# GatorSense/HyperPRI

Hardware: AMD Instinct MI355X
Metric: HSI cubes/sec (608x968x238) fwd+bwd (higher is better)
Workload: dtype f32; 1 GPU; CubeNET-64 n_channels=238 HSI 608x968 fp32, per-GPU batch 2, train mode, BCEWithLogits, fwd+bwd; global_batch=2, parallelism=dp1

## Files before the change

### hyperpri_amd/csrc/common.h

```cpp
#pragma once
#include <hip/hip_runtime.h>
#include <stdint.h>

#define HPRI_OK 0
#define HPRI_ERR_ARG (-1)
#define HPRI_ERR_UNSUPPORTED (-2)
#define HPRI_ERR_WORKSPACE (-3)
#define HPRI_ERR_LAUNCH (-4)

#ifdef HPRI_H16_F16
typedef _Float16 h16_t;
#define HPRI_MFMA_16X16X32 __builtin_amdgcn_mfma_f32_16x16x32_f16
#define HPRI_MFMA_32X32X16 __builtin_amdgcn_mfma_f32_32x32x16_f16
#define HPRI_DS_READ_TR16_B64 __builtin_amdgcn_ds_read_tr16_b64_v4f16
#define HPRI_H16_IS_F16 1
#else
typedef __bf16 h16_t;
#define HPRI_MFMA_16X16X32 __builtin_amdgcn_mfma_f32_16x16x32_bf16
#define HPRI_MFMA_32X32X16 __builtin_amdgcn_mfma_f32_32x32x16_bf16
#define HPRI_DS_READ_TR16_B64 __builtin_amdgcn_ds_read_tr16_b64_v4bf16
#define HPRI_H16_IS_F16 0
#endif

#ifdef HPRI_H16_F16
typedef __fp16 hpri_tr4_t __attribute__((__vector_size__(4 * sizeof(__fp16))));
#else
typedef __bf16 hpri_tr4_t __attribute__((ext_vector_type(4)));
#endif
typedef hpri_tr4_t __attribute__((address_space(3))) * hpri_lds_tr4_ptr;

typedef float f32x16 __attribute__((ext_vector_type(16)));
typedef float f32x4 __attribute__((ext_vector_type(4)));

#define HPRI_CHECK_LAUNCH()                                   \
  do {                                                        \
    hipError_t e__ = hipGetLastError();                       \
    if (e__ != hipSuccess) return hpri_set_error(HPRI_ERR_LAUNCH, hipGetErrorString(e__)); \
  } while (0)

#define HPRI_REQUIRE(cond, msg)                               \
  do {                                                        \
    if (!(cond)) return hpri_set_error(HPRI_ERR_ARG, msg);    \
  } while (0)

int hpri_set_error(int code, const char* msg);
int hpri_option(int idx);
int hpri_cu_count();
float hpri_loss_scale();

static inline int hpri_cdiv(int a, int b) { return (a + b - 1) / b; }
static inline int64_t hpri_cdiv64(int64_t a, int64_t b) { return (a + b - 1) / b; }

enum { HPRI_A_DIRECT = 0, HPRI_A_S2D = 1 };
enum { HPRI_E_DIRECT = 0, HPRI_E_D2S = 1 };

typedef h16_t bf16x4_t __attribute__((ext_vector_type(4)));
struct PlaneOut { h16_t* p; long long plane; int cs, coff, cw, npl; };

#ifdef __HIPCC__
__device__ __forceinline__ void plane_store4(const PlaneOut& pl, size_t pix, int c, float o0, float o1, float o2, float o3) {
  float v[4] = {o0, o1, o2, o3};
  for (int k = 0; k < pl.npl; ++k) {
    bf16x4_t h;
#pragma unroll
    for (int j = 0; j < 4; ++j) { const h16_t t = (h16_t)v[j]; h[j] = t; v[j] -= (float)t; }
    *reinterpret_cast<bf16x4_t*>(pl.p + (size_t)k * pl.plane + pix * pl.cs + pl.coff + c) = h;
  }
}
#endif

#define HPRI_DMA_OOB 0xFFFFFFF0u
#if defined(__HIP_DEVICE_COMPILE__)
typedef __amdgpu_buffer_rsrc_t hpri_rsrc_t;
#define HPRI_MAKE_RSRC(ptr_, bytes_) __builtin_amdgcn_make_buffer_rsrc((void*)(ptr_), 0, (int)(bytes_), 0x00020000)
#define HPRI_LDS_DMA16(rs_, lds_, voff_, soff_) \
  __builtin_amdgcn_raw_ptr_buffer_load_lds(rs_, (__attribute__((address_space(3))) void*)(lds_), 16, voff_, soff_, 0, 0)
#define HPRI_BUFFER_LOAD_F32(rs_, voff_, soff_) __builtin_bit_cast(float, __builtin_amdgcn_raw_buffer_load_b32(rs_, voff_, soff_, 0))
typedef unsigned hpri_u32x4 __attribute__((ext_vector_type(4)));
#define HPRI_BUFFER_LOAD_F32X4(rs_, voff_, soff_) __builtin_bit_cast(f32x4, __builtin_amdgcn_raw_buffer_load_b128(rs_, voff_, soff_, 0))
#define HPRI_BUFFER_STORE_F32X4(v_, rs_, voff_, soff_) \
  __builtin_amdgcn_raw_buffer_store_b128(__builtin_bit_cast(hpri_u32x4, v_), rs_, voff_, soff_, 0)
#else
typedef int hpri_rsrc_t;
#define HPRI_MAKE_RSRC(ptr_, bytes_) 0
#define HPRI_LDS_DMA16(rs_, lds_, voff_, soff_) ((void)(rs_))
#define HPRI_BUFFER_LOAD_F32(rs_, voff_, soff_) 0.f
#define HPRI_BUFFER_LOAD_F32X4(rs_, voff_, soff_) (f32x4{0.f, 0.f, 0.f, 0.f})
#define HPRI_BUFFER_STORE_F32X4(v_, rs_, voff_, soff_) ((void)(rs_))
#endif

#define HPRI_Q_SLICES 8
#define HPRI_Q_STRIDE 1024
#define HPRI_Q_COUNTERS (8 * HPRI_Q_SLICES)
#define HPRI_Q_HALF (HPRI_Q_COUNTERS * HPRI_Q_STRIDE)
#define HPRI_Q_WORDS (2 * HPRI_Q_HALF)
struct HpriQueueHalves { unsigned *use, *clear; };
HpriQueueHalves hpri_item_queue_take(hipStream_t stream);
#ifdef __HIPCC__
__device__ __forceinline__ unsigned hpri_q_draw(unsigned* q, int band, unsigned n) {
  return __hip_atomic_fetch_add(q + band * HPRI_Q_STRIDE, n, __ATOMIC_RELAXED, __HIP_MEMORY_SCOPE_AGENT);
}
__device__ __forceinline__ void hpri_q_clear(unsigned* other, int tid) {
  if (other != nullptr && tid < HPRI_Q_COUNTERS) __hip_atomic_store(other + tid * HPRI_Q_STRIDE, 0u, __ATOMIC_RELAXED, __HIP_MEMORY_SCOPE_AGENT);
}
#endif

static inline int hpri_plane_out(PlaneOut* po, void* planes, long long plane_stride, int pl_cs, int pl_coff, int pl_cw, int npl, int C) {
  po->p = reinterpret_cast<h16_t*>(planes); po->plane = plane_stride; po->cs = pl_cs; po->coff = pl_coff; po->cw = pl_cw; po->npl = npl;
  if (planes == nullptr) { po->cw = 0; po->npl = 0; return HPRI_OK; }
  HPRI_REQUIRE(npl >= 1 && npl <= 3 && pl_cw >= C && pl_cw % 4 == 0 && pl_coff % 4 == 0 && pl_cs % 4 == 0 && pl_coff + pl_cw <= pl_cs &&
                   plane_stride % 4 == 0 && ((uintptr_t)planes & 7) == 0, "bad plane geometry");
  return HPRI_OK;
}
```

### hyperpri_amd/csrc/conv_wino.hip

```cpp
#include "common.h"

typedef float f32x2 __attribute__((ext_vector_type(2)));

extern "C" size_t hpri_wino_packed_floats(int K, int Ncols_pad) { return (size_t)hpri_cdiv(K, 8) * 16 * 8 * Ncols_pad; }

struct WinoWgradArgs {
  const float* x; int x_cs, x_coff, x_cvalid;
  const float* dy; int dy_cs, dy_coff, dy_cvalid;
  float* ws;
  int N, H, W, Cr, Nr, cblk;
  int strips_x, strips_y, total, per_split;
  int ntile, items, per_xcd;
  int kw;
};

#define WG_XROW 36
#define WG_X_BYTES (4 * WG_XROW * 256)
#define WG_Y_BYTES (2 * 32 * 256)
#define WG_STAGE_BYTES (WG_X_BYTES + WG_Y_BYTES)

__global__ __launch_bounds__(512, 2) void conv_wino_wgrad_kernel(WinoWgradArgs a) {
  __shared__ __attribute__((aligned(1024))) unsigned char smem[2 * WG_STAGE_BYTES];
  const int tid = threadIdx.x, lane = tid & 63, wave = __builtin_amdgcn_readfirstlane(tid >> 6);
  const int li = lane & 31, lh = lane >> 5;
  const int fa = wave >> 1, fb = wave & 1;
  const int item = (int)(blockIdx.x & 7) * a.per_xcd + (int)(blockIdx.x >> 3);
  if (item >= a.items) return;
  const int split = item / a.ntile, tile = item - split * a.ntile;
  const int cb = tile % a.cblk, nbk = tile / a.cblk;
  const int c_blk = cb * 64, n_blk = nbk * 64;
  const int u0 = split * a.per_split, u1 = min(a.total, u0 + a.per_split);

  const float s1 = (fa == 2) ? -1.f : 1.f;

  f32x16 acc[2][2][2];
#pragma unroll
  for (int e = 0; e < 2; ++e)
#pragma unroll
    for (int ct = 0; ct < 2; ++ct)
#pragma unroll
      for (int nt = 0; nt < 2; ++nt)
#pragma unroll
        for (int r = 0; r < 16; ++r) acc[e][ct][nt][r] = 0.f;

  constexpr int NPX = 4 * (WG_XROW / 4), NPY = 2 * 8, NPW = (NPX + NPY + 7) / 8;
  constexpr unsigned OOB = 0xFFFFFFF0u;
  const int l4 = lane >> 4;
  const unsigned xlane = (c_blk + (lane & 15) * 4 < a.x_cvalid) ? (unsigned)(l4 * a.x_cs * 4 + (lane & 15) * 16) : OOB;
  const unsigned ylane = (n_blk + (lane & 15) * 4 < a.dy_cvalid) ? (unsigned)(l4 * a.dy_cs * 4 + (lane & 15) * 16) : OOB;
  int ld_sx = u0 % a.strips_x, ld_sy = (u0 / a.strips_x) % a.strips_y, ld_img = u0 / (a.strips_x * a.strips_y);
#define LOAD_UNIT(buf_)                                                                                                \
  {                                                                                                                    \
    const int sx_ = ld_sx, sy_ = ld_sy, img_ = ld_img;                                                                 \
    if (++ld_sx == a.strips_x) { ld_sx = 0; if (++ld_sy == a.strips_y) { ld_sy = 0; ++ld_img; } }                      \
    const int y0_ = sy_ * 2, x0_ = sx_ * 32;                                                                           \
    kend_next = min(8, (a.kw - x0_ + 3) >> 2);                                \
    unsigned char* lb_ = smem + (buf_) * WG_STAGE_BYTES;                                                               \
    const float* xu_ = a.x + ((long long)(img_ * a.H + y0_ - 1) * a.W + x0_ - 1) * a.x_cs + a.x_coff + c_blk;          \
    const float* yu_ = a.dy + ((long long)(img_ * a.H + y0_) * a.W + x0_) * a.dy_cs + a.dy_coff + n_blk;               \
    const hpri_rsrc_t rx_ = HPRI_MAKE_RSRC(xu_, 0x7FFFFF00);       \
    const hpri_rsrc_t ry_ = HPRI_MAKE_RSRC(yu_, 0x7FFFFF00);       \
    _Pragma("unroll") for (int p = 0; p < NPW; ++p) {                                                                  \
      const int piece_ = p * 8 + wave;                                                                                 \
      if (piece_ < NPX) {                                                                                              \
        const int row_ = piece_ / (WG_XROW / 4), pxb_ = (piece_ % (WG_XROW / 4)) * 4;                 \
        const bool rowok_ = (unsigned)(y0_ + row_ - 1) < (unsigned)a.H;                                                \
        const bool ok_ = rowok_ && (pxb_ + l4) < 34 && (unsigned)(x0_ + pxb_ + l4 - 1) < (unsigned)a.W;                \
        HPRI_LDS_DMA16(rx_, lb_ + piece_ * 1024, ok_ ? xlane : OOB, (row_ * a.W + pxb_) * a.x_cs * 4);           \
      } else if (piece_ < NPX + NPY) {                                                                                 \
        const int pp_ = piece_ - NPX;                                                                                  \
        const int row_ = pp_ >> 3, pxb_ = (pp_ & 7) * 4;                                                               \
        const bool ok_ = (y0_ + row_) < a.H && (x0_ + pxb_ + l4) < a.W;                                                \
        HPRI_LDS_DMA16(ry_, lb_ + piece_ * 1024, ok_ ? ylane : OOB, (row_ * a.W + pxb_) * a.dy_cs * 4);          \
      }                                                                                                                \
    }                                                                                                                  \
  }

#define K_STEP(FA_, FB_)                                               \
    {                                                                                                                  \
      constexpr int R1_ = (FA_ == 0) ? 0 : 1, R2_ = (FA_ == 3) ? 3 : 2;              \
      constexpr int YR_ = (FA_ == 3) ? 1 : 0, YROWS_ = (FA_ == 1 || FA_ == 2) ? 2 : 1;                                 \
      asm("" : "+v"(kp));                               \
      f32x2 d[2][3], y[2][2];                                          \
      _Pragma("unroll") for (int c = 0; c < 3; ++c) {                                                                  \
        d[0][c] = WG_LDS2(kp + (R1_ * WG_XROW + FB_ + c) * 256);                                                       \
        d[1][c] = WG_LDS2(kp + (R2_ * WG_XROW + FB_ + c) * 256);                                                       \
      }                                                                                                                \
      _Pragma("unroll") for (int r = 0; r < YROWS_; ++r)                                                               \
        _Pragma("unroll") for (int px = 0; px < 2; ++px) y[r][px] = WG_LDS2(kp + WG_X_BYTES + ((YR_ + r) * 32 + px) * 256); \
      float va[2][2], vb[2][2];                                               \
      float P[3][2];                                                                                                   \
      _Pragma("unroll") for (int c = 0; c < 3; ++c)                                                                    \
        _Pragma("unroll") for (int ct = 0; ct < 2; ++ct) {                                                             \
          float d1_ = d[0][c][ct], d2_ = d[1][c][ct];                                                                  \
          WG_PIN(d1_) WG_PIN(d2_)                                                                                      \
          P[c][ct] = (FA_ == 1) ? (d1_ + d2_) : (d1_ - d2_);                                        \
          WG_PIN(P[c][ct])                                                                                             \
        }                                                                                                              \
      _Pragma("unroll") for (int ct = 0; ct < 2; ++ct) {                                                               \
        va[0][ct] = FB_ ? (P[1][ct] - P[0][ct]) : (P[0][ct] - P[2][ct]);                                               \
        va[1][ct] = FB_ ? (P[0][ct] - P[2][ct]) : (P[1][ct] + P[2][ct]);                                               \
                                                                                                                       \
      }                                                                                                                \
      float t[2][2];                                                               \
      _Pragma("unroll") for (int px = 0; px < 2; ++px)                                                                 \
        _Pragma("unroll") for (int nt = 0; nt < 2; ++nt) {                                                             \
          float y0_ = y[0][px][nt];                                                                                    \
          WG_PIN(y0_)                                                                                                  \
          if (YROWS_ == 2) {                                                                                           \
            float y1_ = y[1][px][nt];                                                                                  \
            WG_PIN(y1_)                                                                                                \
            y0_ = (FA_ == 1) ? (y0_ + y1_) : (y0_ - y1_);                                                              \
            WG_PIN(y0_)                                                                                                \
          }                                                                                                            \
          t[px][nt] = y0_;                                                                                             \
        }                                                                                                              \
      _Pragma("unroll") for (int nt = 0; nt < 2; ++nt) {                                                               \
        vb[0][nt] = FB_ ? (t[0][nt] - t[1][nt]) : t[0][nt];                                                            \
        vb[1][nt] = FB_ ? t[1][nt] : (t[0][nt] + t[1][nt]);                                                            \
                                                                                                                       \
      }                                                                                                                \
      __builtin_amdgcn_sched_barrier(0);                            \
      _Pragma("unroll") for (int e = 0; e < 2; ++e)                                                                    \
          _Pragma("unroll") for (int ct = 0; ct < 2; ++ct)                                                             \
              _Pragma("unroll") for (int nt = 0; nt < 2; ++nt)                                                         \
                  acc[e][ct][nt] = __builtin_amdgcn_mfma_f32_32x32x2f32(va[e][ct], vb[e][nt], acc[e][ct][nt], 0, 0, 0); \
      kp += 1024;                                                                           \
    }
#define UNIT_LOOP(FA_, FB_)                                                                                            \
  for (int u = u0; u < u1; ++u) {                                                                                      \
    asm volatile("s_waitcnt vmcnt(0)" ::: "memory");                                                                   \
    __builtin_amdgcn_s_barrier();                     \
    const int kend = kend_next;                                                                                        \
    if (u + 1 < u1) LOAD_UNIT((u + 1 - u0) & 1)                                                                         \
    unsigned kp = ((u - u0) & 1) * WG_STAGE_BYTES + klane;                                                             \
    for (int kk = 0; kk < kend; ++kk) K_STEP(FA_, FB_)                                                                 \
  }
  const unsigned klane = (unsigned)(lh * 512 + li * 8);
  typedef __attribute__((address_space(3))) const unsigned char* wg_lds_bytes;
  typedef __attribute__((address_space(3))) const volatile f32x2* wg_lds_f32x2;
  const wg_lds_bytes lds = (wg_lds_bytes)smem;
#define WG_LDS2(off_) (*(wg_lds_f32x2)(lds + (off_)))
#define WG_PIN(v_) asm("" : "+v"(v_));
  int kend_next = 8;
  if (u0 < u1) LOAD_UNIT(0)
  switch (wave) {
    case 0: UNIT_LOOP(0, 0) break;
    case 1: UNIT_LOOP(0, 1) break;
    case 2: UNIT_LOOP(1, 0) break;
    case 3: UNIT_LOOP(1, 1) break;
    case 4: UNIT_LOOP(2, 0) break;
    case 5: UNIT_LOOP(2, 1) break;
    case 6: UNIT_LOOP(3, 0) break;
    default: UNIT_LOOP(3, 1) break;
  }
#undef UNIT_LOOP
#undef K_STEP
#undef LOAD_UNIT
#undef WG_LDS2
#undef WG_PIN
  float* slab = a.ws + (size_t)split * 16 * a.Cr * a.Nr;
  const float sdy = (fa == 3) ? -s1 : s1;
  const float sgn[2] = {sdy, (fb == 1) ? -sdy : sdy};
#pragma unroll
  for (int e = 0; e < 2; ++e) {
    const int xi = fa * 4 + 2 * fb + e;
#pragma unroll
    for (int ct = 0; ct < 2; ++ct)
#pragma unroll
      for (int r = 0; r < 16; ++r) {
        const int c = c_blk + 2 * ((r & 3) + 8 * (r >> 2) + 4 * lh) + ct;
        f32x2 o;
        o[0] = sgn[e] * acc[e][ct][0][r];
        o[1] = sgn[e] * acc[e][ct][1][r];
        *reinterpret_cast<f32x2*>(&slab[((size_t)xi * a.Cr + c) * a.Nr + n_blk + 2 * li]) = o;
      }
  }
}

__global__ void wino_wgrad_reduce_kernel(const float* __restrict__ ws, float* __restrict__ dw, int splits, int Cr, int Nr,
                                         int Cin, int Cout, int accumulate) {
  const int n = blockIdx.x * 64 + (threadIdx.x & 63), c = blockIdx.y * 4 + (threadIdx.x >> 6);
  if (n >= Cout || c >= Cin) return;
  float u[16];
#pragma unroll
  for (int xi = 0; xi < 16; ++xi) u[xi] = 0.f;
  const size_t slab = (size_t)16 * Cr * Nr;
  for (int k = 0; k < splits; ++k) {
    const float* p = ws + (size_t)k * slab + (size_t)c * Nr + n;
#pragma unroll
    for (int xi = 0; xi < 16; ++xi) u[xi] += p[(size_t)xi * Cr * Nr];
  }
  float t[3][4];
#pragma unroll
  for (int j = 0; j < 4; ++j) {
    t[0][j] = u[0 * 4 + j] + 0.5f * (u[1 * 4 + j] + u[2 * 4 + j]);
    t[1][j] = 0.5f * (u[1 * 4 + j] - u[2 * 4 + j]);
    t[2][j] = 0.5f * (u[1 * 4 + j] + u[2 * 4 + j]) + u[3 * 4 + j];
  }
  float* o = dw + ((size_t)n * Cin + c) * 9;
#pragma unroll
  for (int i = 0; i < 3; ++i) {
    const float g0 = t[i][0] + 0.5f * (t[i][1] + t[i][2]), g1 = 0.5f * (t[i][1] - t[i][2]), g2 = 0.5f * (t[i][1] + t[i][2]) + t[i][3];
    o[i * 3 + 0] = accumulate ? o[i * 3 + 0] + g0 : g0;
    o[i * 3 + 1] = accumulate ? o[i * 3 + 1] + g1 : g1;
    o[i * 3 + 2] = accumulate ? o[i * 3 + 2] + g2 : g2;
  }
}

constexpr int wino_wide_cols(int S) { return S >= 16 ? 32 : 64; }

template <int S>
__global__ __launch_bounds__(wino_wide_cols(S) * S) void wino_wgrad_reduce_wide_kernel(const float* __restrict__ ws,
                                                                                       float* __restrict__ dw, int splits, int Cr,
                                                                                       int Nr, int Cin, int Cout, int accumulate) {
  constexpr int NC = wino_wide_cols(S);
  __shared__ float red[S - 1][16][NC];
  const int ln = threadIdx.x % NC, sl = threadIdx.x / NC;
  const int n = blockIdx.x * NC + ln, c = blockIdx.y;
  float u[16];
#pragma unroll
  for (int xi = 0; xi < 16; ++xi) u[xi] = 0.f;
  const size_t slab = (size_t)16 * Cr * Nr;
#pragma unroll 1
  for (int k = sl; k < splits; k += S) {
    const float* p = ws + (size_t)k * slab + (size_t)c * Nr + n;
#pragma unroll
    for (int xi = 0; xi < 16; ++xi) u[xi] += p[(size_t)xi * Cr * Nr];
  }
  if (sl > 0) {
#pragma unroll
    for (int xi = 0; xi < 16; ++xi) red[sl - 1][xi][ln] = u[xi];
  }
  __syncthreads();
  if (sl > 0 || n >= Cout) return;
#pragma unroll 2
  for (int q = 0; q < S - 1; ++q)
#pragma unroll
    for (int xi = 0; xi < 16; ++xi) u[xi] += red[q][xi][ln];
  float t[3][4];
#pragma unroll
  for (int j = 0; j < 4; ++j) {
    t[0][j] = u[0 * 4 + j] + 0.5f * (u[1 * 4 + j] + u[2 * 4 + j]);
    t[1][j] = 0.5f * (u[1 * 4 + j] - u[2 * 4 + j]);
    t[2][j] = 0.5f * (u[1 * 4 + j] + u[2 * 4 + j]) + u[3 * 4 + j];
  }
  float* o = dw + ((size_t)n * Cin + c) * 9;
#pragma unroll
  for (int i = 0; i < 3; ++i) {
    const float g0 = t[i][0] + 0.5f * (t[i][1] + t[i][2]), g1 = 0.5f * (t[i][1] - t[i][2]), g2 = 0.5f * (t[i][1] + t[i][2]) + t[i][3];
    o[i * 3 + 0] = accumulate ? o[i * 3 + 0] + g0 : g0;
    o[i * 3 + 1] = accumulate ? o[i * 3 + 1] + g1 : g1;
    o[i * 3 + 2] = accumulate ? o[i * 3 + 2] + g2 : g2;
  }
}

extern "C" int hpri_wino_wgrad_plan(int N, int H, int W, int Cin_pad, int Cout_pad, int* splits, int* Cr, int* Nr) {
  const int cblk = hpri_cdiv(Cin_pad, 64), nblk = hpri_cdiv(Cout_pad, 64);
  const int total = N * hpri_cdiv(H, 2) * hpri_cdiv(W, 32);
  *Cr = cblk * 64; *Nr = nblk * 64;
  const int tiles = cblk * nblk;
  auto plan = [&](int cus, int kmax, double tol) {
    int best = 1; double best_eff = 0.0;
    for (int k = 1; k <= kmax; ++k) {
      if (k > 1 && total / k < 8) break;
      const double per_cu = (double)tiles * k / (double)cus;
      double eff = per_cu / (double)((long long)(per_cu + 0.999999));
      if (per_cu < 1.0) eff = per_cu;
      if (eff > best_eff + tol + 1e-9) { best_eff = eff; best = k; }
    }
    return best;
  };
  int best = plan(256, 512, 0.0);
  const int reserve = hpri_option(5);
  if (reserve > 0) best = plan(256 - (reserve < 192 ? reserve : 192), 2 * best, 0.05);
  *splits = best;
  return HPRI_OK;
}

extern "C" int hpri_conv_wino_wgrad(const float* x, int x_cs, int x_coff, int x_cvalid, const float* dy, int dy_cs, int dy_coff,
                                    int dy_cvalid, float* ws, size_t ws_floats, int N, int H, int W, int Cin_pad, int Cout_pad,
                                    hipStream_t stream) {
  HPRI_REQUIRE(x && dy && ws, "conv_wino_wgrad: null pointer");
  HPRI_REQUIRE(N > 0 && H > 0 && W > 0 && Cin_pad > 0 && Cout_pad > 0, "conv_wino_wgrad: bad sizes");
  HPRI_REQUIRE(x_cs % 4 == 0 && x_coff % 4 == 0 && dy_cs % 4 == 0 && dy_coff % 4 == 0 && x_cvalid % 4 == 0 && dy_cvalid % 4 == 0,
               "conv_wino_wgrad: channel strides / offsets / valid counts must be multiples of 4");
  HPRI_REQUIRE(((uintptr_t)x & 15) == 0 && ((uintptr_t)dy & 15) == 0, "conv_wino_wgrad: pointers must be 16-byte aligned");
  HPRI_REQUIRE((long long)5 * W * x_cs * 4 < (1ll << 31) && (long long)3 * W * dy_cs * 4 < (1ll << 31),
               "conv_wino_wgrad: image rows too long for 32-bit buffer offsets");
  WinoWgradArgs a;
  a.x = x; a.x_cs = x_cs; a.x_coff = x_coff; a.x_cvalid = x_cvalid; a.dy = dy; a.dy_cs = dy_cs; a.dy_coff = dy_coff; a.dy_cvalid = dy_cvalid;
  a.ws = ws; a.N = N; a.H = H; a.W = W;
  int splits;
  hpri_wino_wgrad_plan(N, H, W, Cin_pad, Cout_pad, &splits, &a.Cr, &a.Nr);
  if ((size_t)splits * 16 * a.Cr * a.Nr > ws_floats) return hpri_set_error(HPRI_ERR_WORKSPACE, "conv_wino_wgrad: workspace too small");
  a.cblk = a.Cr / 64;
  a.strips_x = hpri_cdiv(W, 32); a.strips_y = hpri_cdiv(H, 2); a.total = N * a.strips_x * a.strips_y;
  a.per_split = hpri_cdiv(a.total, splits);
  a.ntile = a.cblk * (a.Nr / 64);
  a.items = splits * a.ntile; a.per_xcd = hpri_cdiv(a.items, 8);
  a.kw = hpri_option(6) != 0 ? W : a.strips_x * 32;
  dim3 grid((unsigned)(a.per_xcd * 8), 1u, 1u);
  hipLaunchKernelGGL(conv_wino_wgrad_kernel, grid, dim3(512), 0, stream, a);
  HPRI_CHECK_LAUNCH();
  return HPRI_OK;
}

extern "C" int hpri_wino_wgrad_reduce(const float* ws, float* dw, int N, int H, int W, int Cin, int Cin_pad, int Cout, int Cout_pad,
                                      int accumulate, hipStream_t stream) {
  HPRI_REQUIRE(ws && dw && Cin > 0 && Cout > 0, "wino_wgrad_reduce: bad arguments");
  int splits, Cr, Nr;
  hpri_wino_wgrad_plan(N, H, W, Cin_pad, Cout_pad, &splits, &Cr, &Nr);
  if (splits >= 64) {
    dim3 grid((unsigned)hpri_cdiv(Cout, wino_wide_cols(16)), (unsigned)Cin);
    hipLaunchKernelGGL(wino_wgrad_reduce_wide_kernel<16>, grid, dim3(wino_wide_cols(16) * 16), 0, stream, ws, dw, splits, Cr, Nr, Cin, Cout, accumulate);
  } else if (splits >= 8) {
    dim3 grid((unsigned)hpri_cdiv(Cout, 64), (unsigned)Cin);
    hipLaunchKernelGGL(wino_wgrad_reduce_wide_kernel<8>, grid, dim3(512), 0, stream, ws, dw, splits, Cr, Nr, Cin, Cout, accumulate);
  } else {
    dim3 grid((unsigned)hpri_cdiv(Cout, 64), (unsigned)hpri_cdiv(Cin, 4));
    hipLaunchKernelGGL(wino_wgrad_reduce_kernel, grid, dim3(256), 0, stream, ws, dw, splits, Cr, Nr, Cin, Cout, accumulate);
  }
  HPRI_CHECK_LAUNCH();
  return HPRI_OK;
}
```

Baseline: 68.34 cubes/s.

## Interleave next-unit LDS DMA loads between MFMAs in Winograd wgrad kernel

Restructures the Winograd weight-gradient kernel's prefetch of the next unit. Per-unit buffer load issue is spread across the gaps between the eight MFMAs of the first K step, instead of all being issued up front. Address arithmetic becomes incremental pointer stepping, and boundary handling moves to precomputed per-piece offsets, class-specialised voffsets and resource num_records limits, which replace per-lane bounds checks. This is meant to hide load-issue overhead behind MFMA latency and cut scalar/vector address math. The cost is more code complexity and reliance on buffer descriptor range clamping for correctness at the image edges.

New measurement: 69.18 cubes/s, median of 6. +1.2%, better.

```diff
diff --git a/hyperpri_amd/csrc/common.h b/hyperpri_amd/csrc/common.h
--- a/hyperpri_amd/csrc/common.h
+++ b/hyperpri_amd/csrc/common.h
@@ -82,8 +82,8 @@
   __builtin_amdgcn_raw_buffer_store_b128(__builtin_bit_cast(hpri_u32x4, v_), rs_, voff_, soff_, 0)
 #else
 typedef int hpri_rsrc_t;
-#define HPRI_MAKE_RSRC(ptr_, bytes_) 0
-#define HPRI_LDS_DMA16(rs_, lds_, voff_, soff_) ((void)(rs_))
+#define HPRI_MAKE_RSRC(ptr_, bytes_) ((void)(ptr_), (void)(bytes_), 0)
+#define HPRI_LDS_DMA16(rs_, lds_, voff_, soff_) ((void)(rs_), (void)(lds_), (void)(voff_), (void)(soff_))
 #define HPRI_BUFFER_LOAD_F32(rs_, voff_, soff_) 0.f
 #define HPRI_BUFFER_LOAD_F32X4(rs_, voff_, soff_) (f32x4{0.f, 0.f, 0.f, 0.f})
 #define HPRI_BUFFER_STORE_F32X4(v_, rs_, voff_, soff_) ((void)(rs_))
diff --git a/hyperpri_amd/csrc/conv_wino.hip b/hyperpri_amd/csrc/conv_wino.hip
--- a/hyperpri_amd/csrc/conv_wino.hip
+++ b/hyperpri_amd/csrc/conv_wino.hip
@@ -43,40 +43,69 @@
 #pragma unroll
         for (int r = 0; r < 16; ++r) acc[e][ct][nt][r] = 0.f;
 
-  constexpr int NPX = 4 * (WG_XROW / 4), NPY = 2 * 8, NPW = (NPX + NPY + 7) / 8;
+    constexpr int NPX = 4 * (WG_XROW / 4), NPY = 2 * 8, NPW = (NPX + NPY + 7) / 8;
   constexpr unsigned OOB = 0xFFFFFFF0u;
+  constexpr int NREC = 0x7FFFFF00;
   const int l4 = lane >> 4;
   const unsigned xlane = (c_blk + (lane & 15) * 4 < a.x_cvalid) ? (unsigned)(l4 * a.x_cs * 4 + (lane & 15) * 16) : OOB;
   const unsigned ylane = (n_blk + (lane & 15) * 4 < a.dy_cvalid) ? (unsigned)(l4 * a.dy_cs * 4 + (lane & 15) * 16) : OOB;
-  int ld_sx = u0 % a.strips_x, ld_sy = (u0 / a.strips_x) % a.strips_y, ld_img = u0 / (a.strips_x * a.strips_y);
-#define LOAD_UNIT(buf_)                                                                                                \
+  const unsigned xfirst = l4 >= 1 ? xlane : OOB;
+  const unsigned xtail = l4 < 2 ? xlane : OOB;
+  const int sxl = a.strips_x - 1, syl = a.strips_y - 1, x0l = sxl * 32;
+  const int kend_last = min(8, (a.kw - x0l + 3) >> 2);
+  int ld_sx = u0 % a.strips_x, ld_sy = (u0 / a.strips_x) % a.strips_y;
+  const char *ld_x, *ld_y;
+  {
+    const int img_ = u0 / (a.strips_x * a.strips_y), y0_ = ld_sy * 2, x0_ = ld_sx * 32;
+    ld_x = (const char*)(a.x + ((long long)(img_ * a.H + y0_ - 1) * a.W + x0_ - 1) * a.x_cs + a.x_coff + c_blk);
+    ld_y = (const char*)(a.dy + ((long long)(img_ * a.H + y0_) * a.W + x0_) * a.dy_cs + a.dy_coff + n_blk);
+  }
+  const int px_row = 2 * a.W - x0l, px_img = (a.H - 2 * syl) * a.W - x0l;
+  const int xd_step = 32 * a.x_cs * 4, xd_row = px_row * a.x_cs * 4, xd_img = px_img * a.x_cs * 4;
+  const int yd_step = 32 * a.dy_cs * 4, yd_row = px_row * a.dy_cs * 4, yd_img = px_img * a.dy_cs * 4;
+  int pr_cls, pr_top, pr_bot, pr_bot1, pr_kend;
+  const char *pr_x, *pr_y;
+#define WG_PREPARE                                                                                                     \
   {                                                                                                                    \
-    const int sx_ = ld_sx, sy_ = ld_sy, img_ = ld_img;                                                                 \
-    if (++ld_sx == a.strips_x) { ld_sx = 0; if (++ld_sy == a.strips_y) { ld_sy = 0; ++ld_img; } }                      \
-    const int y0_ = sy_ * 2, x0_ = sx_ * 32;                                                                           \
-    kend_next = min(8, (a.kw - x0_ + 3) >> 2);                                \
-    unsigned char* lb_ = smem + (buf_) * WG_STAGE_BYTES;                                                               \
-    const float* xu_ = a.x + ((long long)(img_ * a.H + y0_ - 1) * a.W + x0_ - 1) * a.x_cs + a.x_coff + c_blk;          \
-    const float* yu_ = a.dy + ((long long)(img_ * a.H + y0_) * a.W + x0_) * a.dy_cs + a.dy_coff + n_blk;               \
-    const hpri_rsrc_t rx_ = HPRI_MAKE_RSRC(xu_, 0x7FFFFF00);       \
-    const hpri_rsrc_t ry_ = HPRI_MAKE_RSRC(yu_, 0x7FFFFF00);       \
-    _Pragma("unroll") for (int p = 0; p < NPW; ++p) {                                                                  \
-      const int piece_ = p * 8 + wave;                                                                                 \
-      if (piece_ < NPX) {                                                                                              \
-        const int row_ = piece_ / (WG_XROW / 4), pxb_ = (piece_ % (WG_XROW / 4)) * 4;                 \
-        const bool rowok_ = (unsigned)(y0_ + row_ - 1) < (unsigned)a.H;                                                \
-        const bool ok_ = rowok_ && (pxb_ + l4) < 34 && (unsigned)(x0_ + pxb_ + l4 - 1) < (unsigned)a.W;                \
-        HPRI_LDS_DMA16(rx_, lb_ + piece_ * 1024, ok_ ? xlane : OOB, (row_ * a.W + pxb_) * a.x_cs * 4);           \
-      } else if (piece_ < NPX + NPY) {                                                                                 \
-        const int pp_ = piece_ - NPX;                                                                                  \
-        const int row_ = pp_ >> 3, pxb_ = (pp_ & 7) * 4;                                                               \
-        const bool ok_ = (y0_ + row_) < a.H && (x0_ + pxb_ + l4) < a.W;                                                \
-        HPRI_LDS_DMA16(ry_, lb_ + piece_ * 1024, ok_ ? ylane : OOB, (row_ * a.W + pxb_) * a.dy_cs * 4);          \
-      }                                                                                                                \
+    const bool lastx_ = ld_sx == sxl, lasty_ = ld_sy == syl;                                                           \
+    pr_cls = lastx_ ? 2 : min(ld_sx, 1);             \
+    pr_kend = lastx_ ? kend_last : 8;                                                                                  \
+    pr_top = ld_sy == 0 ? 0 : NREC;                                                                                    \
+    pr_bot = lasty_ ? 0 : NREC;                                                                                        \
+    pr_bot1 = (lasty_ && (a.H & 1)) ? 0 : NREC;                                                                        \
+    pr_x = ld_x; pr_y = ld_y;                                                                                          \
+    const int xd_ = lastx_ ? (lasty_ ? xd_img : xd_row) : xd_step, yd_ = lastx_ ? (lasty_ ? yd_img : yd_row) : yd_step; \
+    ld_x += xd_; ld_y += yd_;                                                                                          \
+    ld_sx = lastx_ ? 0 : ld_sx + 1;                                                                                    \
+    ld_sy = lastx_ ? (lasty_ ? 0 : ld_sy + 1) : ld_sy;                                                                 \
+  }
+#define WG_PIECE(p_, CLS_)                                                                                             \
+  if ((p_) * 8 + WV_ < NPX + NPY) {                                                                                    \
+    constexpr int piece_ = (p_) * 8 + WV_;                                                                             \
+    constexpr bool isx_ = piece_ < NPX;                                                                                \
+    constexpr int row_ = isx_ ? piece_ / (WG_XROW / 4) : (piece_ - NPX) >> 3;                                          \
+    constexpr int pxb_ = isx_ ? (piece_ % (WG_XROW / 4)) * 4 : ((piece_ - NPX) & 7) * 4;                               \
+    const unsigned vo_ = (CLS_) == 2 ? vlast[p_] : !isx_ ? ylane : pxb_ == 32 ? xtail : ((CLS_) == 0 && pxb_ == 0) ? xfirst : xlane; \
+    const int nrec_ = isx_ ? (row_ == 0 ? pr_top : row_ == 2 ? pr_bot1 : row_ == 3 ? pr_bot : NREC) : (row_ == 1 ? pr_bot1 : NREC); \
+    HPRI_LDS_DMA16(HPRI_MAKE_RSRC(isx_ ? pr_x : pr_y, nrec_), lb_ + piece_ * 1024, vo_, soff[p_]);                     \
+  }
+#define WG_PIECE_SETUP                                                                                                 \
+  int soff[NPW]; unsigned vlast[NPW];                                                                                  \
+  _Pragma("unroll") for (int p = 0; p < NPW; ++p) {                                                                    \
+    const int piece_ = p * 8 + WV_;                                                                                    \
+    soff[p] = 0; vlast[p] = OOB;                                                                                       \
+    if (piece_ < NPX) {                                                                                                \
+      const int row_ = piece_ / (WG_XROW / 4), pxb_ = (piece_ % (WG_XROW / 4)) * 4;                                    \
+      soff[p] = (row_ * a.W + pxb_) * a.x_cs * 4;                                                                      \
+      vlast[p] = ((pxb_ + l4) < 34 && (unsigned)(x0l + pxb_ + l4 - 1) < (unsigned)a.W) ? xlane : OOB;                  \
+    } else if (piece_ < NPX + NPY) {                                                                                   \
+      const int row_ = (piece_ - NPX) >> 3, pxb_ = ((piece_ - NPX) & 7) * 4;                                           \
+      soff[p] = (row_ * a.W + pxb_) * a.dy_cs * 4;                                                                     \
+      vlast[p] = (x0l + pxb_ + l4) < a.W ? ylane : OOB;                                                                \
     }                                                                                                                  \
   }
 
-#define K_STEP(FA_, FB_)                                               \
+#define K_STEP(FA_, FB_, GAP_, END_)         \
     {                                                                                                                  \
       constexpr int R1_ = (FA_ == 0) ? 0 : 1, R2_ = (FA_ == 3) ? 3 : 2;              \
       constexpr int YR_ = (FA_ == 3) ? 1 : 0, YROWS_ = (FA_ == 1 || FA_ == 2) ? 2 : 1;                                 \
@@ -120,22 +149,50 @@
         vb[1][nt] = FB_ ? t[1][nt] : (t[0][nt] + t[1][nt]);                                                            \
                                                                                                                        \
       }                                                                                                                \
+           \
+                   \
+      _Pragma("unroll") for (int e = 0; e < 2; ++e)                                                                    \
+        _Pragma("unroll") for (int q = 0; q < 2; ++q) { asm volatile("" : "+v"(va[e][q])); asm volatile("" : "+v"(vb[e][q])); } \
       __builtin_amdgcn_sched_barrier(0);                            \
-      _Pragma("unroll") for (int e = 0; e < 2; ++e)                                                                    \
-          _Pragma("unroll") for (int ct = 0; ct < 2; ++ct)                                                             \
-              _Pragma("unroll") for (int nt = 0; nt < 2; ++nt)                                                         \
-                  acc[e][ct][nt] = __builtin_amdgcn_mfma_f32_32x32x2f32(va[e][ct], vb[e][nt], acc[e][ct][nt], 0, 0, 0); \
+      WG_MFMA(0, 0, 0) GAP_(0) WG_MFMA(0, 0, 1) GAP_(1) WG_MFMA(0, 1, 0) GAP_(2) WG_MFMA(0, 1, 1) GAP_(3)              \
+      WG_MFMA(1, 0, 0) GAP_(4) WG_MFMA(1, 0, 1) GAP_(5) WG_MFMA(1, 1, 0) GAP_(6) WG_MFMA(1, 1, 1) END_                 \
       kp += 1024;                                                                           \
     }
+#define WG_MFMA(e_, ct_, nt_) \
+  acc[e_][ct_][nt_] = __builtin_amdgcn_mfma_f32_32x32x2f32(va[e_][ct_], vb[e_][nt_], acc[e_][ct_][nt_], 0, 0, 0);
+#define WG_NOGAP(i_)
+#define WG_GAP(i_) __builtin_amdgcn_sched_barrier(0); WG_PIECE_IN_LOOP(i_) __builtin_amdgcn_sched_barrier(0);
+#define WG_END __builtin_amdgcn_sched_barrier(0); kend_next = pr_kend; WG_PREPARE
 #define UNIT_LOOP(FA_, FB_)                                                                                            \
-  for (int u = u0; u < u1; ++u) {                                                                                      \
-    asm volatile("s_waitcnt vmcnt(0)" ::: "memory");                                                                   \
-    __builtin_amdgcn_s_barrier();                     \
-    const int kend = kend_next;                                                                                        \
-    if (u + 1 < u1) LOAD_UNIT((u + 1 - u0) & 1)                                                                         \
-    unsigned kp = ((u - u0) & 1) * WG_STAGE_BYTES + klane;                                                             \
-    for (int kk = 0; kk < kend; ++kk) K_STEP(FA_, FB_)                                                                 \
-  }
+  {                                                                                                                    \
+    constexpr int WV_ = 2 * FA_ + FB_;                                                                                 \
+    WG_PIECE_SETUP                                                                                                     \
+    if (u0 < u1) {                                                                                                     \
+      unsigned char* lb_ = smem;                                                                                       \
+      WG_PREPARE                                                                                                       \
+      kend_next = pr_kend;                                                                                             \
+      WG_PIECE_ANY(0) WG_PIECE_ANY(1) WG_PIECE_ANY(2) WG_PIECE_ANY(3) WG_PIECE_ANY(4) WG_PIECE_ANY(5) WG_PIECE_ANY(6)  \
+      WG_PREPARE                                                                                                       \
+    }                                                                                                                  \
+    for (int u = u0; u < u1; ++u) {                                                                                    \
+      asm volatile("s_waitcnt vmcnt(0)" ::: "memory");                                                                 \
+      __builtin_amdgcn_s_barrier();                   \
+      const int kend = kend_next;                                                                                      \
+      unsigned kp = WG_BUF_OF(u - u0) * WG_STAGE_BYTES + klane;                                                        \
+      int kk = 0;                                                                                                      \
+      if (u + 1 < u1) {                                                                                                \
+        unsigned char* lb_ = smem + ((u + 1 - u0) & 1) * WG_STAGE_BYTES;                                               \
+        K_STEP(FA_, FB_, WG_GAP, WG_END)                                                                               \
+        kk = 1;                                                                                                        \
+      }                                                                                                                \
+      for (; kk < kend; ++kk) K_STEP(FA_, FB_, WG_NOGAP, )                                                             \
+    }                                                                                                                  \
+  }
+#define WG_PIECE_ANY(p_)                                                                                               \
+  if (pr_cls == 2) { WG_PIECE(p_, 2) asm volatile("; last column class"); }                                            \
+  else if (pr_cls == 0 && (p_) * 8 + WV_ < NPX && ((p_) * 8 + WV_) % (WG_XROW / 4) == 0) {                             \
+    WG_PIECE(p_, 0) asm volatile("; first column class");                                                              \
+  } else { WG_PIECE(p_, 1) asm volatile("; middle column class"); }
   const unsigned klane = (unsigned)(lh * 512 + li * 8);
   typedef __attribute__((address_space(3))) const unsigned char* wg_lds_bytes;
   typedef __attribute__((address_space(3))) const volatile f32x2* wg_lds_f32x2;
@@ -143,7 +200,13 @@
 #define WG_LDS2(off_) (*(wg_lds_f32x2)(lds + (off_)))
 #define WG_PIN(v_) asm("" : "+v"(v_));
   int kend_next = 8;
-  if (u0 < u1) LOAD_UNIT(0)
+#ifdef WGRAD_DIAG_NO_UNIT_LOAD
+#define WG_PIECE_IN_LOOP(i_)
+#define WG_BUF_OF(i_) 0
+#else
+#define WG_PIECE_IN_LOOP(i_) WG_PIECE_ANY(i_)
+#define WG_BUF_OF(i_) ((i_) & 1)
+#endif
   switch (wave) {
     case 0: UNIT_LOOP(0, 0) break;
     case 1: UNIT_LOOP(0, 1) break;
@@ -156,7 +219,16 @@
   }
 #undef UNIT_LOOP
 #undef K_STEP
-#undef LOAD_UNIT
+#undef WG_MFMA
+#undef WG_NOGAP
+#undef WG_GAP
+#undef WG_END
+#undef WG_PIECE_ANY
+#undef WG_PIECE_IN_LOOP
+#undef WG_PIECE
+#undef WG_PIECE_SETUP
+#undef WG_PREPARE
+#undef WG_BUF_OF
 #undef WG_LDS2
 #undef WG_PIN
   float* slab = a.ws + (size_t)split * 16 * a.Cr * a.Nr;
```
